# imuncle/TSCM_Calib

Measured on AMD Instinct MI355X. Metric: LM iterations/sec at 4 cams x 10k views (joint intrinsics+extrinsics, fp64), higher is better.
Workload: dtype f64

## Files before the change

### tscm_calib_amd/csrc/tscm_kernels.h

```cpp
#pragma once

#include "tscm_math.h"
#include "tscm_fastmath.h"
#include "tscm_nd_plan.h"
#include "tscm_layout.h"
#include "tscm_exec_plan.h"
#include "tscm_columns.h"
#include "tscm_ctrl.h"

namespace tscm {

static_assert(kColFree == kFA && kColGrad == kFR, "tscm_columns.h plans the columns of tscm_math.h's camera tile");
constexpr int kWcolTc = 3;
constexpr int kFac = 56;
constexpr int kFacM = 0;
constexpr int kFacC = 15;
constexpr int kFacL = 21;
constexpr int kFacI = 36;
constexpr int kFacZ = 42;
constexpr int kFacD = 48;
constexpr int kTcols = 15;
constexpr int kTcWb = 0, kTcWc = 4, kTcF = 8, kTcOne = 9, kTcXi = 10, kTcLam = 12, kTcAl = 13, kTcR = 14;
__host__ __device__ constexpr int tc_tc(int j) { return 3 + 4 * j; }
constexpr int kVConst = 27;
constexpr int kCConst = 48;
constexpr int kCStride = 72;
constexpr int kCst = 80;
constexpr int kScal = 8;
constexpr int kStStride = 16;

#if defined(TSCM_PHASE_PROFILE) || defined(TSCM_WAVE_TIMELINE)
#define PHASE_STAMP(var) const long long var = wall_clock64()
#else
#define PHASE_STAMP(var)
#endif

__device__ __forceinline__ void wave_lds_fence()
{
    __builtin_amdgcn_fence(__ATOMIC_RELEASE, "wavefront");
    __builtin_amdgcn_wave_barrier();
    __builtin_amdgcn_fence(__ATOMIC_ACQUIRE, "wavefront");
}

typedef int v2i __attribute__((ext_vector_type(2)));
__device__ __forceinline__ __amdgpu_buffer_rsrc_t make_rsrc(const void *p, size_t bytes)
{
    return __builtin_amdgcn_make_buffer_rsrc(const_cast<void *>(p), 0, (int)(bytes > 0xffffffffull ? 0xffffffffu : (unsigned)bytes), 0x00020000);
}
__device__ __forceinline__ double buf_load_f64(__amdgpu_buffer_rsrc_t r, unsigned voff, unsigned soff)
{
    return __builtin_bit_cast(double, __builtin_amdgcn_raw_buffer_load_b64(r, (int)voff, (int)soff, 0));
}
#ifndef TSCM_STORE_AUX
#define TSCM_STORE_AUX 0
#endif
__device__ __forceinline__ void buf_store_f64(__amdgpu_buffer_rsrc_t r, unsigned voff, unsigned soff, double v)
{
    __builtin_amdgcn_raw_buffer_store_b64(__builtin_bit_cast(v2i, v), r, (int)voff, (int)soff, TSCM_STORE_AUX);
}

typedef double d4 __attribute__((ext_vector_type(4)));
typedef double d2 __attribute__((ext_vector_type(2)));
typedef int v4i __attribute__((ext_vector_type(4)));
__device__ __forceinline__ d2 buf_load_2f64(__amdgpu_buffer_rsrc_t r, unsigned voff, unsigned soff)
{
    return __builtin_bit_cast(d2, __builtin_amdgcn_raw_buffer_load_b128(r, (int)voff, (int)soff, 0));
}
__device__ __forceinline__ void buf_store_2f64(__amdgpu_buffer_rsrc_t r, unsigned voff, double a, double b)
{
    const d2 v = { a, b };
    __builtin_amdgcn_raw_buffer_store_b128(__builtin_bit_cast(v4i, v), r, (int)voff, 0, TSCM_STORE_AUX);
}

#ifndef TSCM_PRIO
#define TSCM_PRIO 10
#endif
__device__ __forceinline__ void set_prio(int p)
{
    switch (p & 3) {
    case 0: __builtin_amdgcn_s_setprio(0); break;
    case 1: __builtin_amdgcn_s_setprio(1); break;
    case 2: __builtin_amdgcn_s_setprio(2); break;
    default: __builtin_amdgcn_s_setprio(3); break;
    }
}

__device__ __forceinline__ const double *rec_w(const double *rec, int slot) { return rec + (size_t)kRecW * slot; }
__device__ __forceinline__ const double *rec_e(const double *rec, int V, int slot) { return rec + (size_t)kRecW * V + (size_t)kRecE * slot; }
__device__ __forceinline__ const double *rec_g(const double *rec, int V, int slot) { return rec + (size_t)(kRecW + kRecE) * V + (size_t)kRecG * slot; }

struct Ctrl : CtrlHead {
    IterLog log[kMaxLog];
};

struct DevProblem {
    int C, B, n_points, V, N, n_pad;
    int n_chunks, n_pchunks, n_bids;
    int rp, half;
    int lds_wave;
    const double *board_xy;
    const int *view_cam, *view_board, *view_obs, *view_count;
    const double *obs_u, *obs_v;
    const int *chunk_vb, *chunk_ve, *chunk_cam, *cam_chunk_ptr;
    const int4 *chunk_desc;
    const int *bv_ptr;
    const int *view_slot, *slot_cam;
    const int *slot_view, *slot_board;
    const int *slow_boards;
    int n_slow;
    const int *pair_i, *pair_j;
    const int *pc_begin, *pc_end, *pc_tile;
    const int *bid_part_ptr;
    const int *pair_board;
    const int *bc_tile;
    const int4 *bc_desc;
    int n_bchunks, n_tiles;
    const unsigned char *col_ctl;
    const unsigned char *board_const;
    const unsigned char *col_active;
    const int *act_map;
    int n_act;
    int cam_pre[9];
    unsigned short cam_free[8];
    unsigned long long pair_mask;
    const int4 *solve_map;
    int cam_wg[9];
    int rank, world;
    const short *bid_lut;
    int bid_part_small[kSmallBids + 1];
    int g4_per;
};

struct DevState {
    double *cam_rt[2], *intr[2], *board_rt[2];
    double *board_pc, *cam_pc;
    double *vconst;
    double *cconst[2];
    double *rec[2];
    double *campart, *campart2;
    double *H[2], *H_stage;
    double *s_b, *s_c;
    double *fac;
    double *pairpart, *T;
    int *t_count;
    int *fac_fail;
    int *y_flag;
    double *yhat;
    double *Abig;
    double *bs_part, *st_part;
    int n_bs_blocks, n_st_blocks;
    Ctrl *ctrl;
    CtrlHead *ctrl_snap;
    int *stats_count, *stats_flag;
    struct CtlPub *ctl_pub;
};
struct CtlPub { int epoch, cur, done, pad; double radius; };

__global__ void k_pose_prep(DevProblem P, DevState S, int cand)
{
    if (S.ctrl->done) return;
    const int tgt = cand ? (S.ctrl->cur ^ 1) : S.ctrl->cur;
    const int i = blockIdx.x * blockDim.x + threadIdx.x;
    if (i < P.B) {
        double rt[6], out[kBoardConst];
        for (int k = 0; k < 6; ++k) rt[k] = S.board_rt[tgt][6 * i + k];
        board_constants(rt, out);
        for (int k = 0; k < kBoardConst; ++k) S.board_pc[(size_t)kBoardConst * i + k] = out[k];
    } else if (i < P.B + P.C) {
        const int m = i - P.B;
        double rt[6], out[kCamConst];
        for (int k = 0; k < 6; ++k) rt[k] = S.cam_rt[tgt][6 * m + k];
        camera_constants(rt, out);
        for (int k = 0; k < kCamConst; ++k) S.cam_pc[kCamConst * m + k] = out[k];
    }
}

__device__ __forceinline__ void load_view_const(const DevProblem &P, const DevState &S, int tgt, int cam, int board, ViewConst &vc)
{
    const double *bp = S.board_pc + (size_t)kBoardConst * board;
    for (int k = 0; k < 3; ++k) { vc.r1[k] = bp[k]; vc.r2[k] = bp[3 + k]; vc.tb[k] = S.board_rt[tgt][6 * board + 3 + k]; }
    for (int k = 0; k < 3; ++k) for (int q = 0; q < 6; ++q) vc.db[k][q] = bp[6 + 6 * k + q];
    const double *cp = S.cam_pc + kCamConst * cam;
    for (int k = 0; k < 9; ++k) vc.Rc[k] = cp[k];
    for (int k = 0; k < 27; ++k) vc.dRc[k] = cp[9 + k];
    for (int k = 0; k < 3; ++k) vc.tc[k] = S.cam_rt[tgt][6 * cam + 3 + k];
    const double *I = S.intr[tgt] + 9 * cam;
    vc.fx = I[0]; vc.fy = I[1]; vc.cx = I[2]; vc.cy = I[3]; vc.xi = I[4]; vc.lam = I[5]; vc.al = I[6];
}

__device__ __forceinline__ void view_point_constants(const double Rc[9], const double *tc, const double *bc , const double *tb, double *o)
{
    for (int r = 0; r < 3; ++r) {
        o[r] = Rc[3 * r] * bc[0] + Rc[3 * r + 1] * bc[1] + Rc[3 * r + 2] * bc[2];
        o[3 + r] = Rc[3 * r] * bc[3] + Rc[3 * r + 1] * bc[4] + Rc[3 * r + 2] * bc[5];
        o[6 + r] = (Rc[3 * r] * tb[0] + Rc[3 * r + 1] * tb[1] + Rc[3 * r + 2] * tb[2]) + tc[r];
    }
}

#if defined(__HIP_DEVICE_COMPILE__) && !defined(__gfx950__) && !defined(__gfx942__)
#error "the in-launch hand-offs (handoff_store / handoff_load) rely on gfx942 / gfx950 sc1 write-through semantics: re-derive them for this target"
#endif
constexpr long long kHandoffTimeoutTicks = 50 * 1000 * 1000;
__device__ __forceinline__ void handoff_store(double *p, double v) { __hip_atomic_store(p, v, __ATOMIC_RELAXED, __HIP_MEMORY_SCOPE_AGENT); }
__device__ __forceinline__ double handoff_load(const double *p) { return __hip_atomic_load(p, __ATOMIC_RELAXED, __HIP_MEMORY_SCOPE_AGENT); }

__device__ __forceinline__ void write_camera_record(const DevState &S, int tgt, int m, const double *cam_rt, const double *intr)
{
    double crt[3], Rc[9], a[9], wsm[3];
    for (int k = 0; k < 3; ++k) crt[k] = cam_rt[6 * m + k];
    const int small = camera_rotation_constants(crt, Rc, a, wsm);
    double *o = S.cconst[tgt] + kCStride * m;
    for (int k = 0; k < 9; ++k) o[k] = Rc[k];
    for (int k = 0; k < 3; ++k) o[9 + k] = cam_rt[6 * m + 3 + k];
    for (int k = 0; k < 9; ++k) o[12 + k] = a[k];
    for (int k = 0; k < 3; ++k) o[21 + k] = wsm[k];
    o[24] = small ? 1.0 : 0.0;
    for (int k = 25; k < 39; ++k) o[k] = 0.0;
    double I[7];
    for (int k = 0; k < 7; ++k) I[k] = intr[9 * m + k];
    for (int k = 0; k < 6; ++k) o[39 + k] = I[k];
    const double oma = 1.0 - I[6];
    o[45] = I[6] / oma;
    o[46] = 1.0 / (oma * oma);
    o[47] = 0.0;
    float *of = reinterpret_cast<float *>(o + kCConst);
    for (int k = 0; k < kCConst; ++k) of[k] = (float)o[k];
}
__device__ __forceinline__ void write_camera_record(const DevState &S, int tgt, int m) { write_camera_record(S, tgt, m, S.cam_rt[tgt], S.intr[tgt]); }

constexpr int kVStride = 48;
constexpr int kVFloatOff = 32;

__device__ __forceinline__ void view_prep_body(const DevProblem &P, const DevState &S, int tgt, int with_floats, const double *cam_rt, const double *intr, const double *board_rt)
{
    __shared__ double st[kVPrepThreads][kVFloatOff + 1];
    const int t = threadIdx.x;
    const int i = blockIdx.x * kVPrepThreads + t;
    if (i < P.V) {
        const int b = P.view_board[i], m = P.view_cam[i];
        double rt[6], bc[kBoardConst], Rc[9], dRc[27];
        for (int k = 0; k < 6; ++k) rt[k] = board_rt[6 * b + k];
        board_constants(rt, bc);
        double crt[3];
        for (int k = 0; k < 3; ++k) crt[k] = cam_rt[6 * m + k];
        rotation_and_derivatives(crt, Rc, dRc);
        double *o = st[t];
        view_point_constants(Rc, cam_rt + 6 * m + 3, bc, rt + 3, o);
        for (int k = 0; k < 6; ++k) {
            const double d0 = bc[6 + 3 * k], d1 = bc[6 + 3 * k + 1], d2 = bc[6 + 3 * k + 2];
            for (int r = 0; r < 3; ++r) o[9 + 3 * k + r] = Rc[3 * r] * d0 + Rc[3 * r + 1] * d1 + Rc[3 * r + 2] * d2;
        }
        for (int k = kVConst; k < kVFloatOff; ++k) o[k] = 0.0;
    } else if (i < P.V + P.C) {
        write_camera_record(S, tgt, i - P.V, cam_rt, intr);
    }
    __syncthreads();
    const int v0 = blockIdx.x * kVPrepThreads;
    const int nv = min(kVPrepThreads, P.V - v0);
    for (int e = t; e < nv * kVFloatOff; e += kVPrepThreads) {
        const int v = e / kVFloatOff, k = e % kVFloatOff;
        S.vconst[(size_t)kVStride * (v0 + v) + k] = st[v][k];
    }
    if (with_floats) {
        constexpr int kF = kVStride - kVFloatOff;
        for (int e = t; e < nv * kF; e += kVPrepThreads) {
            const int v = e / kF, k = e % kF, j = 2 * k;
            const float f0 = j < kVConst ? (float)st[v][j] : 0.f, f1 = j + 1 < kVConst ? (float)st[v][j + 1] : 0.f;
            S.vconst[(size_t)kVStride * (v0 + v) + kVFloatOff + k] = __hiloint2double(__float_as_int(f1), __float_as_int(f0));
        }
    }
}

__global__ __launch_bounds__(kVPrepThreads) void k_view_prep(DevProblem P, DevState S, int cand, int with_floats)
{
    if (S.ctrl->done) return;
    const int tgt = cand ? (S.ctrl->cur ^ 1) : S.ctrl->cur;
    view_prep_body(P, S, tgt, with_floats, S.cam_rt[tgt], S.intr[tgt], S.board_rt[tgt]);
}

__host__ __device__ __forceinline__ constexpr int f_tile(int f)
{
    return f < 3 ? kTcWc + f : f < 6 ? tc_tc(f - 3) : f < 8 ? kTcF : f < 10 ? kTcOne : f == 10 ? kTcXi : f == 11 ? kTcLam : f == 12 ? kTcAl : kTcR;
}
__device__ __forceinline__ int f_mask(int f) { return (f >= 6 && f < 10) ? (1 << ((f - 6) & 1)) : 3; }

typedef const double __attribute__((address_space(4))) *cptr4;

struct RecLane { unsigned off, stride, goff, gstride; };
__device__ __forceinline__ RecLane rec_lane(int lane, unsigned V)
{
    const int col = lane & 15, kq = lane >> 4;
    RecLane r;
    r.goff = col == kTcR ? 8u * ((unsigned)(kRecW + kRecE) * V + (unsigned)kq) : 0xffffe000u; r.gstride = col == kTcR ? 8u * kRecG : 0u;
    if (col < 3) { r.off = 8u * ((unsigned)kRecW * V + 6u * (unsigned)col + (unsigned)kq); r.stride = 8u * kRecE; }
    else if (col == 15) { r.off = 0xffffe000u; r.stride = 0u; }
    else {
        const int f = (col & 3) == 3 ? kWcolTc + (col >> 2) : col < 8 ? col - kTcWc : col == kTcF ? 6 : col == kTcOne ? 8 : col == kTcXi ? 10 : col - 1;
        r.off = 8u * (6u * (unsigned)f + (unsigned)kq); r.stride = 8u * kRecW;
    }
    return r;
}

template <typename PW, typename PR>
__host__ __device__ __forceinline__ double tb_tb(PW W, PR Rc, int l, int lp)
// ... 1285 lines not shown
#pragma unroll
            for (int b = 0; b < kFA; ++b) o.hrow[b] = H[256 * m + ai * 16 + b];
            o.hg = H[256 * m + ai * 16 + kFR];
        }
    }
}
__device__ __forceinline__ void reduced_solution_tail(const DevProblem &P, const DevState &S, int cur, int fail, const TailOperands &o,
                                                      const double *yv, const double *s_sc, double *s_yh, const unsigned char *s_act, double *sred,
                                                      int publish_epoch = 0)
{
    const int n = P.n_pad, i = threadIdx.x;
    const int m = i >> 4, ai = i & 15;
    double model = 0.0, stepsq = 0.0, yh = 0.0;
    if (i < n) {
        const bool act = s_act[i] && !fail;
        yh = act ? s_sc[i] * yv[i] : 0.0;
        handoff_store(&S.yhat[i], yh);
        s_yh[i] = yh;
        if (ai < kFA) {
            const double x = o.x;
            const double xn = x + (-yh);
            if (ai < 6) handoff_store(&S.cam_rt[cur ^ 1][6 * m + ai], xn); else handoff_store(&S.intr[cur ^ 1][9 * m + (ai - 6)], xn);
            const double d = x - xn; stepsq = d * d;
        } else if (ai < 15) {
            handoff_store(&S.intr[cur ^ 1][9 * m + (ai - 6)], o.x);
        }
    }
    if (publish_epoch > 0) asm volatile("s_waitcnt vmcnt(0)" ::: "memory");
    __syncthreads();
    if (publish_epoch > 0 && i == 0) __hip_atomic_store(S.y_flag, 2 * publish_epoch + (fail ? 1 : 0), __ATOMIC_RELAXED, __HIP_MEMORY_SCOPE_AGENT);
    if (publish_epoch > 0 && i >= 64 && i < 64 + P.C) write_camera_record(S, cur ^ 1, i - 64);
    if (i < n && ai < kFA && yh != 0.0) {
        double hy = 0.0;
#pragma unroll
        for (int b = 0; b < kFA; ++b) hy += o.hrow[b] * s_yh[m * 16 + b];
        model = yh * (o.hg - 0.5 * hy);
    }
    { double red[2] = { model, stepsq }, mdummy = 0.0; block_reduce256<2>(red, mdummy, sred); model = red[0]; stepsq = red[1]; }
    if (i == 0) { S.ctrl->model_cam = model; S.ctrl->stepsq_cam = stepsq; S.ctrl->lin_fail = fail; *S.fac_fail = 0; }
}

template <int NTH, bool WAIT>
__device__ __forceinline__ void backsub_body(const DevProblem &P, const DevState &S, int with_floats, const int blk, const int nblk, const int epoch, const int t_need);

#include "tscm_solve_nd.h"
#include "tscm_solve_dense4.h"

constexpr int kBigNT = 1024;
constexpr int kBigBatch = 4;
__host__ __device__ inline size_t solve_big_lds_bytes(int N, int n_pad)
{
    return sizeof(double) * ((size_t)2 * 16 * (N + 16) + 16 * 17 + 2 * (size_t)N + 16 + 3 * (size_t)n_pad) + sizeof(int) * (size_t)N + (size_t)n_pad;
}
__device__ __forceinline__ size_t big_block(int I, int J) { return ((size_t)(I * (I + 1) / 2 + J)) << 8; }
__device__ __forceinline__ size_t big_idx(int r, int c)
{
    return big_block(r >> 4, c >> 4) + (size_t)((((c & 15) + 16 * (r & 3)) << 2) + ((r & 15) >> 2));
}
__device__ __forceinline__ double readlane_f64(double v, int lane)
{
    return __hiloint2double(__builtin_amdgcn_readlane(__double2hiint(v), lane), __builtin_amdgcn_readlane(__double2loint(v), lane));
}
__device__ __forceinline__ void lds_barrier() { asm volatile("s_waitcnt lgkmcnt(0)\n\ts_barrier" ::: "memory"); }

__global__ __launch_bounds__(kBigNT) void k_solve_reduced_big(DevProblem P, DevState S)
{
    extern __shared__ __attribute__((aligned(32))) double lds[];
    const int n = P.n_pad, na = P.n_act;
    const int N = (na + 15) & ~15, NP = N >> 4;
    const int XP = N + 16;
    double *pbuf = lds;
    double *Ld = pbuf + 2 * 16 * XP;
    double *wv = Ld + 16 * 17;
    double *idg = wv + N;
    double *yk = idg + N;
    double *yv = yk + 16;
    double *s_sc = yv + n;
    double *s_yh = s_sc + n;
    int *s_map = reinterpret_cast<int *>(s_yh + n);
    unsigned char *s_act = reinterpret_cast<unsigned char *>(s_map + N);
    __shared__ int s_fail;
    __shared__ double sred[256];
    const int tid = threadIdx.x, wave = tid >> 6, lane = tid & 63;
    if (S.ctrl->done) return;
    const int cur = S.ctrl->cur;
    const double radius = S.ctrl->radius;
    const double dmin = S.ctrl->opt.min_lm_diagonal, dmax = S.ctrl->opt.max_lm_diagonal;
    const double *H = S.H[cur];
    double *A = S.Abig;
    for (int i = tid; i < n; i += kBigNT) { s_sc[i] = S.s_c[i]; s_act[i] = P.col_active[i]; yv[i] = 0.0; }
    for (int i = tid; i < N; i += kBigNT) s_map[i] = i < na ? P.act_map[i] : -1;
    if (tid == 0) s_fail = S.ctrl->lin_fail | *S.fac_fail;
    __syncthreads();
#ifdef TSCM_BIG_PROFILE
    long long tp0 = wall_clock64(), tp_diag = 0, tp_solve = 0, tp_upd = 0;
#endif
    for (int kb = 0; wave + 16 * kb <= N; kb += 16) {
        const int rmax = min(N, wave + 16 * (kb + 15));
        for (int c = lane; c <= rmax && c < N; c += 64) {
            const int j = s_map[c];
            const int mj = j >> 4, bj = j & 15;
            const double scj = j >= 0 ? s_sc[j] : 0.0;
            double v[16];
#pragma unroll
            for (int u = 0; u < 16; ++u) {
                const int r = wave + 16 * (kb + u);
                v[u] = (r == c) ? 1.0 : 0.0;
                if (r > N || c > r) continue;
                if (r == N) {
                    v[u] = j >= 0 ? scj * (H[256 * mj + bj * 16 + kFR] - load_T_lut(P, S.T, j, mj * 16 + kFR)) : 0.0;
                } else {
                    const int i = s_map[r];
                    if (i >= 0 && j >= 0) {
                        const int mi = i >> 4, ai = i & 15;
                        const double h = (mi == mj) ? H[256 * mi + ai * 16 + bj] : 0.0;
                        double t = s_sc[i] * scj * (h - load_T_lut(P, S.T, i, j));
                        if (i == j) t += fmin(fmax(scj * scj * h, dmin), dmax) / radius;
                        v[u] = t;
                    }
                }
            }
#pragma unroll
            for (int u = 0; u < 16; ++u) {
                const int r = wave + 16 * (kb + u);
                if (r > N || c > r) continue;
                if (c < 16) pbuf[c * XP + r] = v[u];
                else A[big_idx(r, c)] = v[u];
            }
        }
    }
    __syncthreads();
#ifdef TSCM_BIG_PROFILE
    long long tp1 = wall_clock64();
#endif
    for (int tk = 0; tk < NP; ++tk) {
        const int k0 = tk * 16, m0 = k0 + 16;
        double *pc = pbuf + (tk & 1) * (16 * XP);
        double *pn = pbuf + ((tk & 1) ^ 1) * (16 * XP);
#ifdef TSCM_BIG_PROFILE
        const long long q0 = wall_clock64();
#endif
        if (wave == 0) {
            const int r = lane & 15;
            double a[16];
#pragma unroll
            for (int c = 0; c < 16; ++c) a[c] = pc[c * XP + r];
#pragma unroll
            for (int c = 0; c < 16; ++c) {
                double d = readlane_f64(a[c], c);
                if (!(d > 0.0)) { d = 1.0; if (lane == 0) s_fail = 1; }
                const double isd = fast_rsqrt(d);
                const double l = a[c] * isd;
                a[c] = l;
                if (lane == c) idg[k0 + c] = isd;
#pragma unroll
                for (int q = c + 1; q < 16; ++q) a[q] -= l * readlane_f64(l, q);
            }
            if (lane < 16) {
#pragma unroll
                for (int c = 0; c < 16; ++c) if (c <= r) { Ld[r * 17 + c] = a[c]; A[big_idx(k0 + r, k0 + c)] = a[c]; }
            }
        }
        lds_barrier();
#ifdef TSCM_BIG_PROFILE
        const long long q1 = wall_clock64();
#endif
        for (int r = m0 + tid; r <= N; r += kBigNT) {
            double x[16];
#pragma unroll
            for (int c = 0; c < 16; ++c) x[c] = pc[c * XP + (r - k0)];
#pragma unroll
            for (int c = 0; c < 16; ++c) {
                double v = x[c];
#pragma unroll
                for (int q = 0; q < c; ++q) v -= x[q] * Ld[c * 17 + q];
                x[c] = v * idg[k0 + c];
            }
#pragma unroll
            for (int c = 0; c < 16; ++c) { A[big_idx(r, k0 + c)] = x[c]; pc[c * XP + (r - k0)] = x[c]; }
        }
        lds_barrier();
#ifdef TSCM_BIG_PROFILE
        const long long q2 = wall_clock64();
#endif
        {
            const int col = lane & 15, kq = lane >> 4;
            const int Tb = tk + 1;
            for (int I = Tb + (((wave >> 2) - Tb) & 3); I <= NP; I += 4) {
                double xa[4];
#pragma unroll
                for (int t = 0; t < 4; ++t) xa[t] = -pc[(4 * t + kq) * XP + (16 * I - k0) + col];
                for (int J0 = Tb + (((wave & 3) - Tb) & 3); J0 <= I && J0 < NP; J0 += 4 * kBigBatch) {
                    d4 acc[kBigBatch];
#pragma unroll
                    for (int u = 0; u < kBigBatch; ++u) {
                        const int J = J0 + 4 * u;
                        const int Jc = (J <= I && J < NP) ? J : J0;
                        acc[u] = *reinterpret_cast<const d4 *>(A + big_block(I, Jc) + 4 * lane);
                    }
#pragma unroll
                    for (int u = 0; u < kBigBatch; ++u) {
                        const int J = J0 + 4 * u;
                        if (!(J <= I && J < NP)) continue;
                        double xb[4];
#pragma unroll
                        for (int t = 0; t < 4; ++t) xb[t] = pc[(4 * t + kq) * XP + (16 * J - k0) + col];
#pragma unroll
                        for (int t = 0; t < 4; ++t) acc[u] = __builtin_amdgcn_mfma_f64_16x16x4f64(xa[t], xb[t], acc[u], 0, 0, 0);
                    }
#pragma unroll
                    for (int u = 0; u < kBigBatch; ++u) {
                        const int J = J0 + 4 * u;
                        if (!(J <= I && J < NP)) continue;
                        if (J == Tb) {
#pragma unroll
                            for (int g = 0; g < 4; ++g) pn[col * XP + 16 * (I - Tb) + kq + 4 * g] = acc[u][g];
                        } else {
                            *reinterpret_cast<d4 *>(A + big_block(I, J) + 4 * lane) = acc[u];
                        }
                    }
                }
            }
        }
        lds_barrier();
#ifdef TSCM_BIG_PROFILE
        { const long long q3 = wall_clock64(); tp_diag += q1 - q0; tp_solve += q2 - q1; tp_upd += q3 - q2; }
#endif
    }
    __syncthreads();
#ifdef TSCM_BIG_PROFILE
    long long tp2 = wall_clock64();
#endif
    for (int i = tid; i < N; i += kBigNT) wv[i] = A[big_idx(N, i)];
    double lrow[16], ldg[4];
    {
        const int k0 = (NP - 1) * 16;
#pragma unroll
        for (int c = 0; c < 16; ++c) lrow[c] = (NP > 0 && tid < k0) ? A[big_idx(k0 + c, tid)] : 0.0;
#pragma unroll
        for (int u = 0; u < 4; ++u) { const int e = lane + 64 * u, r = e >> 4, c = e & 15; ldg[u] = (NP > 0 && wave == 0 && c <= r) ? A[big_idx(k0 + r, k0 + c)] : 0.0; }
    }
    __syncthreads();
    for (int tk = NP - 1; tk >= 0; --tk) {
        const int k0 = tk * 16;
        double lnext[16], dnext[4];
        {
            const int kn = k0 - 16;
#pragma unroll
            for (int c = 0; c < 16; ++c) lnext[c] = (tk > 0 && tid < kn) ? A[big_idx(kn + c, tid)] : 0.0;
#pragma unroll
            for (int u = 0; u < 4; ++u) { const int e = lane + 64 * u, r = e >> 4, c = e & 15; dnext[u] = (tk > 0 && wave == 0 && c <= r) ? A[big_idx(kn + r, kn + c)] : 0.0; }
        }
        if (wave == 0) {
#pragma unroll
            for (int u = 0; u < 4; ++u) { const int e = lane + 64 * u; Ld[(e >> 4) * 17 + (e & 15)] = ldg[u]; }
            wave_lds_fence();
            if (lane == 0) {
                double y[16];
#pragma unroll
                for (int c = 15; c >= 0; --c) {
                    double v = wv[k0 + c];
#pragma unroll
                    for (int q = c + 1; q < 16; ++q) v -= Ld[q * 17 + c] * y[q];
                    y[c] = v * idg[k0 + c];
                }
#pragma unroll
                for (int c = 0; c < 16; ++c) { yk[c] = y[c]; wv[k0 + c] = y[c]; }
            }
        }
        lds_barrier();
        if (tid < k0) {
            double v = wv[tid];
#pragma unroll
            for (int c = 0; c < 16; ++c) v -= lrow[c] * yk[c];
            wv[tid] = v;
        }
        lds_barrier();
#pragma unroll
        for (int c = 0; c < 16; ++c) lrow[c] = lnext[c];
#pragma unroll
        for (int u = 0; u < 4; ++u) ldg[u] = dnext[u];
    }
    TailOperands tail_ops;
    tail_prefetch(P, S, cur, H, tail_ops);
    for (int i = tid; i < na; i += kBigNT) yv[s_map[i]] = wv[i];
    __syncthreads();
#ifdef TSCM_BIG_PROFILE
    long long tp3 = wall_clock64();
#endif
    reduced_solution_tail(P, S, cur, s_fail, tail_ops, yv, s_sc, s_yh, s_act, sred);
#ifdef TSCM_BIG_PROFILE
    if (tid == 0) printf("big solve N=%d  build %lld  factor %lld (diag %lld solve %lld update %lld)  backsub %lld  tail %lld  [10 ns ticks]\n", N,
                         tp1 - tp0, tp2 - tp1, tp_diag, tp_solve, tp_upd, tp3 - tp2, wall_clock64() - tp3);
#endif
}

constexpr int kBsTile = 64;
template <int NTH> struct BsGeom {
    static constexpr int kBoards = NTH / 8;
    static constexpr int kPassSlots = NTH / 16;
    static constexpr int kPasses = 4;
    static constexpr int kRoundSlots = kPasses * kPassSlots;
    static constexpr int kLdsA = kRoundSlots * 6, kLdsB = kBoards * kFac, kLdsC = kBsTile * (kVFloatOff + 1);
    static constexpr int kLds = kLdsC > kLdsB ? (kLdsC > kLdsA ? kLdsC : kLdsA) : (kLdsB > kLdsA ? kLdsB : kLdsA);
    static_assert(kBoards * kFac == 7 * NTH, "the factor records are 7 doubles per thread");
    static_assert(kBoards <= 64 && 64 + kMaxCam <= NTH, "lane roles of phase B: the boards in wave 0, the cameras from wave 1 on");
};

template <int NTH, bool WAIT>
__device__ __forceinline__ void backsub_body(const DevProblem &P, const DevState &S, int with_floats, const int blk, const int nblk, const int epoch, const int t_need)
{
    constexpr int kBsBoards = BsGeom<NTH>::kBoards, kBsThreads = NTH, kPassSlots = BsGeom<NTH>::kPassSlots, kPasses = BsGeom<NTH>::kPasses, kRoundSlots = BsGeom<NTH>::kRoundSlots;
#ifndef TSCM_BS_CAM_LANE0
#define TSCM_BS_CAM_LANE0 64
#endif
    constexpr int kBsCamLane0 = TSCM_BS_CAM_LANE0;
    const int b0 = blk * kBsBoards;
    const int nbl = min(kBsBoards, P.B - b0);
    const int s0 = P.bv_ptr[b0], s1 = P.bv_ptr[b0 + nbl];
    const int ctrl_done = S.ctrl->done, cur = S.ctrl->cur;
    int fail = WAIT ? 0 : S.ctrl->lin_fail;
    if (ctrl_done) return;
    extern __shared__ __attribute__((aligned(16))) double dyn[];
    double (*s_qv)[6] = reinterpret_cast<double (*)[6]>(dyn);
    double *s_fac = dyn;
    double *st_all = dyn;
    __shared__ double s_q[kBsBoards][6], s_new[kBsBoards][6];
    __shared__ double s_yh[16 * kMaxCam];
    double (*s_rc)[12] = reinterpret_cast<double (*)[12]>(s_yh);
    static_assert(12 * kMaxCam <= 16 * kMaxCam, "s_rc aliases s_yh");
    __shared__ double sm[16];
    __shared__ int s_view[kBsTile];
    const int t = threadIdx.x;
    PHASE_STAMP(ts0);
    const int my_q0 = t < nbl ? P.bv_ptr[b0 + t] : 0, my_q1 = t < nbl ? P.bv_ptr[b0 + t + 1] : 0;
    const int c_slot = min(s0 + t, max(s1 - 1, 0));
    const int c_view = s1 > s0 ? P.slot_view[c_slot] : 0, c_board = s1 > s0 ? P.slot_board[c_slot] : 0, c_cam = s1 > s0 ? P.slot_cam[c_slot] : 0;
    double xb[6], sbv[6];
#pragma unroll
    for (int k = 0; k < 6; ++k) { xb[k] = t < nbl ? S.board_rt[cur][6 * (b0 + t) + k] : 0.0; sbv[k] = t < nbl ? S.s_b[6 * (b0 + t) + k] : 1.0; }
    double facv[7];
#pragma unroll
    for (int j = 0; j < 7; ++j) facv[j] = S.fac[(size_t)kFac * b0 + min(t + kBsThreads * j, nbl * kFac - 1)];
    if constexpr (!WAIT) { for (int i = t; i < P.n_pad; i += kBsThreads) s_yh[i] = S.yhat[i]; }
    if (t < kBsBoards * 6) (&s_q[0][0])[t] = 0.0;
    if constexpr (!WAIT) { if (t == 64) for (int m = blk; m < P.C; m += nblk) write_camera_record(S, cur ^ 1, m); }
    {
        const int grp = t >> 4, a = t & 15;
        const __amdgpu_buffer_rsrc_t r_w = make_rsrc(S.rec[cur], sizeof(double) * (size_t)kRecW * P.V);
        constexpr unsigned BAD = 0xffffe000u;
        double w[kPasses][6];
        int camv[kPasses];
        auto request = [&](int rbase) {
#pragma unroll
            for (int j = 0; j < kPasses; ++j) {
                const int slot = rbase + kPassSlots * j + grp;
                const unsigned off = (a < kFA && slot < s1) ? 8u * ((unsigned)kRecW * (unsigned)slot + 6u * (unsigned)a) : BAD;
#pragma unroll
                for (int k = 0; k < 3; ++k) { const d2 v = buf_load_2f64(r_w, off, 16u * (unsigned)k); w[j][2 * k] = v[0]; w[j][2 * k + 1] = v[1]; }
                camv[j] = P.slot_cam[min(slot, max(s1 - 1, 0))];
            }
        };
        request(s0);
        if constexpr (WAIT) {
            __shared__ int s_flag;
            if (t == 0) {
                const long long t_start = wall_clock64();
                int f;
                while (((f = __hip_atomic_load(S.y_flag, __ATOMIC_RELAXED, __HIP_MEMORY_SCOPE_AGENT)) >> 1) < epoch) {
                    __builtin_amdgcn_s_sleep(8);
                    if (wall_clock64() - t_start > kHandoffTimeoutTicks) { f = -1; break; }
                }
                if (f < 0) {
                    __hip_atomic_store(&S.ctrl->fault, 1, __ATOMIC_RELAXED, __HIP_MEMORY_SCOPE_AGENT);
                    __hip_atomic_store(&S.ctrl->term_type, 2, __ATOMIC_RELAXED, __HIP_MEMORY_SCOPE_AGENT);
                    __hip_atomic_store(&S.ctrl->done, 1, __ATOMIC_RELAXED, __HIP_MEMORY_SCOPE_AGENT);
                }
                s_flag = f;
            }
            __syncthreads();
            if (s_flag < 0 || __hip_atomic_load(&S.ctrl->done, __ATOMIC_RELAXED, __HIP_MEMORY_SCOPE_AGENT)) return;
            fail = s_flag & 1;
            for (int i = t; i < P.n_pad; i += kBsThreads) s_yh[i] = handoff_load(&S.yhat[i]);
        }
        for (int rbase = s0; rbase < s1; rbase += kRoundSlots) {
            const int rend = min(s1, rbase + kRoundSlots);
            __syncthreads();
#pragma unroll
            for (int j = 0; j < kPasses; ++j) {
                const int sl = kPassSlots * j + grp;
                const double yh = a < kFA ? s_yh[16 * camv[j] + a] : 0.0;
                double p[6];
#pragma unroll
                for (int k = 0; k < 6; ++k) {
                    p[k] = (a < kFA ? w[j][k] : 0.0) * yh;
                    p[k] = row16_allsum(p[k]);
                }
                if (a == 0) {
#pragma unroll
                    for (int k = 0; k < 6; ++k) s_qv[sl][k] = p[k];
                }
            }
            if (rbase + kRoundSlots < s1) request(rbase + kRoundSlots);
            __syncthreads();
            if (t < nbl) {
                for (int q = max(my_q0, rbase); q < min(my_q1, rend); ++q)
#pragma unroll
                    for (int k = 0; k < 6; ++k) s_q[t][k] += s_qv[q - rbase][k];
            }
        }
        __syncthreads();
#pragma unroll
        for (int j = 0; j < 7; ++j) s_fac[t + kBsThreads * j] = facv[j];
        __syncthreads();
    }
    PHASE_STAMP(ts1);
    double mb = 0.0, ss = 0.0;
    if (t < nbl) {
        const int b = b0 + t;
        if (my_q1 == my_q0 || fail) {
#pragma unroll
            for (int k = 0; k < 6; ++k) { S.board_rt[cur ^ 1][6 * b + k] = xb[k]; s_new[t][k] = xb[k]; }
        } else {
            const double *f = s_fac + kFac * t;
            double tt[6], y[6], pz[6];
#pragma unroll
            for (int i = 0; i < 6; ++i) {
                double v = f[kFacC + i] * s_q[t][i];
#pragma unroll
                for (int k = 0; k < i; ++k) v -= f[kFacM + i * (i - 1) / 2 + k] * pz[k];
                pz[i] = v;
                tt[i] = f[kFacZ + i] - v;
            }
#pragma unroll
            for (int i = 5; i >= 0; --i) {
                double w = tt[i];
#pragma unroll
                for (int k = i + 1; k < 6; ++k) w -= f[kFacL + k * (k - 1) / 2 + i] * y[k];
                y[i] = w * f[kFacI + i];
            }
#pragma unroll
            for (int k = 0; k < 6; ++k) {
                mb += 0.5 * tt[k] * tt[k] + 0.5 * f[kFacD + k] * y[k] * y[k];
                const double x = xb[k];
                const double xn = x + (-(sbv[k] * y[k]));
                const double d = x - xn;
                ss += d * d;
                S.board_rt[cur ^ 1][6 * b + k] = xn;
                s_new[t][k] = xn;
            }
        }
    } else if (t >= kBsCamLane0 && t < kBsCamLane0 + P.C) {
        const int m = t - kBsCamLane0;
        double crt[3], Rc[9], dRc[27];
        double crt6[6];
#pragma unroll
        for (int k = 0; k < 6; ++k) crt6[k] = WAIT ? handoff_load(&S.cam_rt[cur ^ 1][6 * m + k]) : S.cam_rt[cur ^ 1][6 * m + k];
        for (int k = 0; k < 3; ++k) crt[k] = crt6[k];
        rotation_and_derivatives(crt, Rc, dRc);
        for (int k = 0; k < 9; ++k) s_rc[m][k] = Rc[k];
        for (int k = 0; k < 3; ++k) s_rc[m][9 + k] = crt6[3 + k];

    }
    {
        double red[2] = { mb, ss }, mdummy = 0.0;
        block_reduce256<2>(red, mdummy, sm);
        if (t == 0) { S.bs_part[2 * blk] = red[0]; S.bs_part[2 * blk + 1] = red[1]; }
    }
    PHASE_STAMP(ts2);
    for (int base = s0; base < s1; base += kBsTile) {
        const int slot = base + t;
        int view = -1;
        if (t < kBsTile && slot < s1) {
            const bool first = base == s0;
            view = first ? c_view : P.slot_view[slot];
            const int bl = (first ? c_board : P.slot_board[slot]) - b0, m = first ? c_cam : P.slot_cam[slot];
            double rt[6], bc[kBoardConst];
#pragma unroll
            for (int k = 0; k < 6; ++k) rt[k] = s_new[bl][k];
            board_constants(rt, bc);
            double *o = st_all + (size_t)t * (kVFloatOff + 1);
            view_point_constants(s_rc[m], s_rc[m] + 9, bc, rt + 3, o);
            for (int k = 0; k < 6; ++k) {
                const double d0 = bc[6 + 3 * k], d1 = bc[6 + 3 * k + 1], d2 = bc[6 + 3 * k + 2];
                for (int r = 0; r < 3; ++r) o[9 + 3 * k + r] = s_rc[m][3 * r] * d0 + s_rc[m][3 * r + 1] * d1 + s_rc[m][3 * r + 2] * d2;
            }
            for (int k = kVConst; k < kVFloatOff; ++k) o[k] = 0.0;
        }
        if (t < kBsTile) s_view[t] = view;
        __syncthreads();
        const int nrec = min(kBsTile, s1 - base);
        for (int e = t; e < nrec * kVFloatOff; e += kBsThreads) {
            const int v = e / kVFloatOff, k = e % kVFloatOff;
            S.vconst[(size_t)kVStride * s_view[v] + k] = st_all[(size_t)v * (kVFloatOff + 1) + k];
        }
        if (with_floats) {
            constexpr int kF = kVStride - kVFloatOff;
            for (int e = t; e < nrec * kF; e += kBsThreads) {
                const int v = e / kF, k = e % kF, j = 2 * k;
                const double *sv = st_all + (size_t)v * (kVFloatOff + 1);
                const float f0 = j < kVConst ? (float)sv[j] : 0.f, f1 = j + 1 < kVConst ? (float)sv[j + 1] : 0.f;
                S.vconst[(size_t)kVStride * s_view[v] + kVFloatOff + k] = __hiloint2double(__float_as_int(f1), __float_as_int(f0));
            }
        }
        __syncthreads();
    }
#ifdef TSCM_WAVE_TIMELINE
    if (threadIdx.x == 0 && S.ctrl->iteration == 5 && blk < kKtlGroups) {
        long long *o = g_phs + (size_t)kPhStamps * (kKtlGroups + blk);
        o[0] = ts0; o[1] = ts0; o[2] = ts1; o[3] = ts2; o[4] = wall_clock64(); o[5] = o[4]; o[6] = nbl; o[7] = 0;
    }
#endif
#ifdef TSCM_PHASE_PROFILE
    if (threadIdx.x == 0 && (blk == 0 || blk == 200))
        printf("backsub_prep wg %d: W.yhat %lld  board solve %lld  view constants %lld [10 ns]\n", blk, ts1 - ts0, ts2 - ts1, wall_clock64() - ts2);
#endif
}

template <int NTH>
__global__ __launch_bounds__(NTH) void k_backsub_prep(DevProblem P, DevState S, int with_floats)
{
    KTL(5);
    backsub_body<NTH, false>(P, S, with_floats, (int)blockIdx.x, (int)gridDim.x, 0, 0);
}

__device__ void control_step(const DevProblem &P, const DevState &S, int init, const ControlPre &pre, double *sm, const double *H, const double *sc, double *stage_copy,
                             bool writer, CtlOut *out)
{
    Ctrl &g = *S.ctrl;
    CtrlHead c = pre.c;
    const int t = threadIdx.x;
    if (out && t == 0) { out->cur = c.cur; out->done = c.done; out->radius = c.radius; out->dmin = c.opt.min_lm_diagonal; out->dmax = c.opt.max_lm_diagonal; }
    if (c.done) return;
    const Options &o = c.opt;
    const int tgt = init ? c.cur : (c.cur ^ 1);
    double gmax_c = 0.0, gsq_c = 0.0, xsq_c = 0.0, cost = 0.0;
#pragma unroll
    for (int j = 0; j < 2; ++j) {
        const int p = t + 256 * j;
        if (p >= 16 * P.C) break;
        const int m = p >> 4, a = p & 15;
        if (pre.free_param[j]) {
            const double x = pre.x[j];
            const double g = pre.grad_param[j] ? H[256 * m + a * 16 + kFR] : 0.0;
            const double d = x - (x + (-g));
            gmax_c = fmax(gmax_c, fabs(d)); gsq_c += d * d; xsq_c += x * x;
        }
        if (a == 15) cost += 0.5 * H[256 * m + kFR * 16 + kFR];
        if (init && writer && a < 15) {
            const double hii = (a < kFA) ? H[256 * m + a * 16 + a] : 0.0;
            S.s_c[p] = o.jacobi_scaling ? 1.0 / (1.0 + sqrt(hii)) : 1.0;
        }
        if (init && writer && a == 15) S.s_c[p] = 1.0;
    }
    KTLX(4, true);
    { double red[3] = { gsq_c, xsq_c, cost }; block_reduce256<3>(red, gmax_c, sm); gsq_c = red[0]; xsq_c = red[1]; cost = red[2]; }
    KTLX(5, true);
    if (writer) {
#pragma unroll 8
        for (int i = t; i < 256 * P.C; i += 256) { const double h = H[i]; S.H[tgt][i] = h; if (stage_copy) stage_copy[i] = h; }
        if (stage_copy && t < kScal + P.world) stage_copy[256 * P.C + t] = sc[t];
    }
    if (t != 0) return;
    auto commit = [&]() {
        c.fin_count = 0;
        if (writer) static_cast<CtrlHead &>(g) = c;
        if (out) { out->cur = c.cur; out->done = c.done; out->radius = c.radius; }
    };
    double gmax_b = 0.0;
    for (int r = 0; r < P.world; ++r) gmax_b = fmax(gmax_b, sc[kScal + r]);
    const double gmax_t = fmax(gmax_c, gmax_b);
    if (sc[4] > 0.0) c.lin_fail = 1;
    const double gnorm_t = sqrt(gsq_c + sc[3]);
    const double xnorm_t = sqrt(xsq_c + sc[2]);
    KTLX(6, true);

    IterLog it;
    const StepInput in = { cost, gmax_t, gnorm_t, xnorm_t, sc[0] + c.model_cam, sqrt(sc[1] + c.stepsq_cam) };
    if (lm_step(c, init, tgt, in, it) && writer && c.n_log <= kMaxLog) g.log[c.n_log - 1] = it;
    commit();
}

__global__ __launch_bounds__(256) void k_control(DevProblem P, DevState S, int init)
{
    __shared__ double sm[256];
    ControlPre pre;
    control_prefetch(P, S, init, pre, S.ctrl);
    control_step(P, S, init, pre, sm, S.H_stage, S.H_stage + 256 * P.C, nullptr);
}

__global__ __launch_bounds__(kVPrepThreads) void k_begin_view_prep(DevProblem P, DevState S, CtrlHead head, const double *src_cam, const double *src_intr,
                                                                   const double *src_board, double *bak_cam, double *bak_intr, double *bak_board, int with_floats)
{
    const int i0 = blockIdx.x * kVPrepThreads + threadIdx.x, n = gridDim.x * kVPrepThreads;
    if (i0 == 0) { head.t_begin = wall_clock64(); static_cast<CtrlHead &>(*S.ctrl) = head; }
    if (i0 == 0) { *S.t_count = 0; *S.y_flag = 0; *S.fac_fail = 0; S.ctl_pub->epoch = 0; *S.stats_count = 0; *S.stats_flag = 0; }
    const double *cam = src_cam ? src_cam : S.cam_rt[0], *intr = src_intr ? src_intr : S.intr[0], *board = src_board ? src_board : S.board_rt[0];
    for (int i = i0; i < 6 * P.C; i += n) { const double v = cam[i]; if (src_cam) S.cam_rt[0][i] = v; if (bak_cam) bak_cam[i] = v; }
    for (int i = i0; i < 9 * P.C; i += n) { const double v = intr[i]; if (src_intr) S.intr[0][i] = v; if (bak_intr) bak_intr[i] = v; }
    for (int i = i0; i < 6 * P.B; i += n) { const double v = board[i]; if (src_board) S.board_rt[0][i] = v; if (bak_board) bak_board[i] = v; }
    view_prep_body(P, S, 0, with_floats, cam, intr, board);
}

__global__ __launch_bounds__(256) void k_end_solve(DevState S, int C, int B)
{
    const int i0 = blockIdx.x * 256 + threadIdx.x, n = gridDim.x * 256;
    if (i0 == 0) S.ctrl->t_end = wall_clock64();
    if (S.ctrl->cur == 0) return;
    for (int i = i0; i < 6 * C; i += n) S.cam_rt[0][i] = S.cam_rt[1][i];
    for (int i = i0; i < 9 * C; i += n) S.intr[0][i] = S.intr[1][i];
    for (int i = i0; i < 6 * B; i += n) S.board_rt[0][i] = S.board_rt[1][i];
}

__global__ __launch_bounds__(256) void k_finish_solve(DevProblem P, DevState S, int init, int have_backsub, int C, int B, Ctrl *host_ctrl)
{
    constexpr int kHl = 256 * kMaxCamLds + kScal + 8, kGall = 512 * kMaxCamLds;
    __shared__ double sm[256];
    __shared__ double Hl[kHl];
    __shared__ CtlOut s_ctl;
    const CtrlHead *head = S.ctrl_snap;
    if (blockIdx.x == 0) {
        __shared__ double Gall[kGall];
        finish_evaluation<false>(P, S, init, have_backsub, true, Hl, Gall, sm, &s_ctl, head);
        __syncthreads();
        if (threadIdx.x == 0) S.ctrl->t_end = wall_clock64();
        __threadfence();
        __syncthreads();
        const int n_log = min(max(__hip_atomic_load(&S.ctrl->n_log, __ATOMIC_RELAXED, __HIP_MEMORY_SCOPE_AGENT), 0), kMaxLog);
        const int words = (int)((sizeof(CtrlHead) + sizeof(IterLog) * (size_t)n_log) / 8);
        const unsigned long long *src = reinterpret_cast<const unsigned long long *>(S.ctrl);
        unsigned long long *dst = reinterpret_cast<unsigned long long *>(host_ctrl);
        for (int i = threadIdx.x; i < words; i += 256) dst[i] = __hip_atomic_load(&src[i], __ATOMIC_RELAXED, __HIP_MEMORY_SCOPE_AGENT);
        return;
    }
    control_outcome(P, S, init, have_backsub, Hl, sm, &s_ctl, head);
    __syncthreads();
    if (__builtin_amdgcn_readfirstlane(s_ctl.cur) == 0) return;
    const int i0 = (blockIdx.x - 1) * 256 + threadIdx.x, n = (gridDim.x - 1) * 256;
    for (int i = i0; i < 6 * C; i += n) S.cam_rt[0][i] = S.cam_rt[1][i];
    for (int i = i0; i < 9 * C; i += n) S.intr[0][i] = S.intr[1][i];
    for (int i = i0; i < 6 * B; i += n) S.board_rt[0][i] = S.board_rt[1][i];
}

__global__ void k_eval_functor(DevProblem P, DevState S, const int *corner_view, double *res,
                               double *Jc, double *Jb, double *Ji)
{
    const int k = blockIdx.x * blockDim.x + threadIdx.x;
    if (k >= P.N) return;
    const int view = corner_view[k];
    const int j = k - P.view_obs[view];
    ViewConst vc;
    load_view_const(P, S, 0, P.view_cam[view], P.view_board[view], vc);
    double r[2], JE[2][kE], JF[2][kFA];
    corner_residual_jacobian(vc, P.board_xy[2 * j], P.board_xy[2 * j + 1], P.obs_u[k], P.obs_v[k], r, JE, JF);
    res[2 * k] = r[0]; res[2 * k + 1] = r[1];
    for (int row = 0; row < 2; ++row) {
        if (Jc) for (int i = 0; i < 6; ++i) Jc[12 * (size_t)k + 6 * row + i] = JF[row][i];
        if (Jb) for (int i = 0; i < 6; ++i) Jb[12 * (size_t)k + 6 * row + i] = JE[row][i];
        if (Ji) { for (int i = 0; i < 7; ++i) Ji[18 * (size_t)k + 9 * row + i] = JF[row][6 + i]; Ji[18 * (size_t)k + 9 * row + 7] = 0.0; Ji[18 * (size_t)k + 9 * row + 8] = 0.0; }
    }
}

__global__ __launch_bounds__(64) void k_reproj_error(DevProblem P, const double *cam_rt, const double *intr,
                                                    const double *board_rt, double *view_err, double *view_sq)
{
    const int view = blockIdx.x, lane = threadIdx.x;
    const int cam = P.view_cam[view], board = P.view_board[view];
    double Rb[9], Rc[9], dummy[27], I[9];
    rotation_and_derivatives(board_rt + 6 * board, Rb, dummy);
    rotation_and_derivatives(cam_rt + 6 * cam, Rc, dummy);
    for (int i = 0; i < 9; ++i) I[i] = intr[9 * cam + i];
    const double *tb = board_rt + 6 * board + 3, *tc = cam_rt + 6 * cam + 3;
    double e = 0.0, sq = 0.0;
    for (int j = lane; j < P.view_count[view]; j += 64) {
        const double x = P.board_xy[2 * j], y = P.board_xy[2 * j + 1];
        double q[3], Pc[3];
        for (int i = 0; i < 3; ++i) q[i] = Rb[3 * i] * x + Rb[3 * i + 1] * y + tb[i];
        for (int i = 0; i < 3; ++i) Pc[i] = Rc[3 * i] * q[0] + Rc[3 * i + 1] * q[1] + Rc[3 * i + 2] * q[2] + tc[i];
        double u, v;
        project_point(I, Pc[0], Pc[1], Pc[2], u, v);
        const double du = P.obs_u[P.view_obs[view] + j] - u, dv = P.obs_v[P.view_obs[view] + j] - v;
        e += sqrt(du * du + dv * dv); sq += du * du + dv * dv;
    }
    for (int s = 32; s > 0; s >>= 1) { e += __shfl_xor(e, s); sq += __shfl_xor(sq, s); }
    if (lane == 0) { view_err[view] = e; view_sq[view] = sq; }
}

__global__ void k_project(const double *intr, const double *pts, int n, double *uv)
{
    const int i = blockIdx.x * blockDim.x + threadIdx.x;
    if (i >= n) return;
    double I[9];
    for (int k = 0; k < 9; ++k) I[k] = intr[k];
    project_point(I, pts[3 * i], pts[3 * i + 1], pts[3 * i + 2], uv[2 * i], uv[2 * i + 1]);
}

__global__ void k_unproject(const double *intr, const double *uv, int n, double *rays)
{
    const int i = blockIdx.x * blockDim.x + threadIdx.x;
    if (i >= n) return;
    double I[9], r[3];
    for (int k = 0; k < 9; ++k) I[k] = intr[k];
    unproject_pixel(I, uv[2 * i], uv[2 * i + 1], r);
    rays[3 * i] = r[0]; rays[3 * i + 1] = r[1]; rays[3 * i + 2] = r[2];
}

}
```

Baseline: 8718.

## Split view-record construction across waves and precompute board constants once per board

```diff
diff --git a/tscm_calib_amd/csrc/tscm_kernels.h b/tscm_calib_amd/csrc/tscm_kernels.h
--- a/tscm_calib_amd/csrc/tscm_kernels.h
+++ b/tscm_calib_amd/csrc/tscm_kernels.h
@@ -1,5 +1,6 @@
 #pragma once
 
+#include <type_traits>
 #include "tscm_math.h"
 #include "tscm_fastmath.h"
 #include "tscm_nd_plan.h"
@@ -1891,10 +1892,30 @@
     static constexpr int kPasses = 4;
     static constexpr int kRoundSlots = kPasses * kPassSlots;
     static constexpr int kLdsA = kRoundSlots * 6, kLdsB = kBoards * kFac, kLdsC = kBsTile * (kVFloatOff + 1);
-    static constexpr int kLds = kLdsC > kLdsB ? (kLdsC > kLdsA ? kLdsC : kLdsA) : (kLdsB > kLdsA ? kLdsB : kLdsA);
+    static constexpr int kLdsABC = kLdsC > kLdsB ? (kLdsC > kLdsA ? kLdsC : kLdsA) : (kLdsB > kLdsA ? kLdsB : kLdsA);
+    static constexpr int kBcPitch = kBoardConst + 1, kLdsBc = kBoards * kBcPitch;
+    static constexpr int kLds = kLdsABC + kLdsBc;
+    static constexpr int kWaves = NTH / 64;
+    static constexpr int kBcWave = kWaves >= 3 ? 2 : 0, kPoseWave = kWaves - 1;
     static_assert(kBoards * kFac == 7 * NTH, "the factor records are 7 doubles per thread");
     static_assert(kBoards <= 64 && 64 + kMaxCam <= NTH, "lane roles of phase B: the boards in wave 0, the cameras from wave 1 on");
+    static_assert(kBcWave != 1 && kPoseWave != kBcWave, "the board constants are formed next to the camera rotations (wave 1) and the pose stores");
 };
+template <int NW> struct BsRoles;
+template <> struct BsRoles<4> { static constexpr int kLo[5] = { 0, 9, 15, 21, kVConst }; };
+template <> struct BsRoles<2> { static constexpr int kLo[3] = { 0, 15, kVConst }; };
+template <int NW> constexpr bool bs_roles_cover()
+{
+    int seen[kVConst] = {};
+    for (int w = 0; w < NW; ++w) {
+        const int lo = BsRoles<NW>::kLo[w], hi = BsRoles<NW>::kLo[w + 1];
+        if (lo % 3 || hi % 3 || (lo > 0 && lo < 9)) return false;
+        for (int k = lo; k < hi; ++k) { if (k < 0 || k >= kVConst) return false; ++seen[k]; }
+    }
+    for (int k = 0; k < kVConst; ++k) if (seen[k] != 1) return false;
+    return true;
+}
+static_assert(bs_roles_cover<4>() && bs_roles_cover<2>(), "every output 0 .. 26 of a view record belongs to exactly one wave");
 
 template <int NTH, bool WAIT>
 __device__ __forceinline__ void backsub_body(const DevProblem &P, const DevState &S, int with_floats, const int blk, const int nblk, const int epoch, const int t_need)
@@ -1914,6 +1935,8 @@
     double (*s_qv)[6] = reinterpret_cast<double (*)[6]>(dyn);
     double *s_fac = dyn;
     double *st_all = dyn;
+    double *s_bc = dyn + BsGeom<NTH>::kLdsABC;
+    constexpr int kBcPitch = BsGeom<NTH>::kBcPitch, kWaves = BsGeom<NTH>::kWaves;
     __shared__ double s_q[kBsBoards][6], s_new[kBsBoards][6];
     __shared__ double s_yh[16 * kMaxCam];
     double (*s_rc)[12] = reinterpret_cast<double (*)[12]>(s_yh);
@@ -1921,10 +1944,15 @@
     __shared__ double sm[16];
     __shared__ int s_view[kBsTile];
     const int t = threadIdx.x;
+    const int wv = __builtin_amdgcn_readfirstlane(t >> 6), ln = t & 63;
     PHASE_STAMP(ts0);
     const int my_q0 = t < nbl ? P.bv_ptr[b0 + t] : 0, my_q1 = t < nbl ? P.bv_ptr[b0 + t + 1] : 0;
-    const int c_slot = min(s0 + t, max(s1 - 1, 0));
-    const int c_view = s1 > s0 ? P.slot_view[c_slot] : 0, c_board = s1 > s0 ? P.slot_board[c_slot] : 0, c_cam = s1 > s0 ? P.slot_cam[c_slot] : 0;
+    int c_view = 0, c_board = 0, c_cam = 0, n_view = 0, n_board = 0, n_cam = 0;
+    auto request_tile = [&](int base, int &view, int &board, int &cam) {
+        const int slot = min(base + ln, s1 - 1);
+        view = P.slot_view[slot]; board = P.slot_board[slot]; cam = P.slot_cam[slot];
+    };
+    if (s1 > s0) { request_tile(s0, c_view, c_board, c_cam); request_tile(s0 + kBsTile, n_view, n_board, n_cam); }
     double xb[6], sbv[6];
 #pragma unroll
     for (int k = 0; k < 6; ++k) { xb[k] = t < nbl ? S.board_rt[cur][6 * (b0 + t) + k] : 0.0; sbv[k] = t < nbl ? S.s_b[6 * (b0 + t) + k] : 1.0; }
@@ -2006,10 +2034,9 @@
     PHASE_STAMP(ts1);
     double mb = 0.0, ss = 0.0;
     if (t < nbl) {
-        const int b = b0 + t;
         if (my_q1 == my_q0 || fail) {
 #pragma unroll
-            for (int k = 0; k < 6; ++k) { S.board_rt[cur ^ 1][6 * b + k] = xb[k]; s_new[t][k] = xb[k]; }
+            for (int k = 0; k < 6; ++k) s_new[t][k] = xb[k];
         } else {
             const double *f = s_fac + kFac * t;
             double tt[6], y[6], pz[6];
@@ -2035,7 +2062,6 @@
                 const double xn = x + (-(sbv[k] * y[k]));
                 const double d = x - xn;
                 ss += d * d;
-                S.board_rt[cur ^ 1][6 * b + k] = xn;
                 s_new[t][k] = xn;
             }
         }
@@ -2051,31 +2077,55 @@
         for (int k = 0; k < 3; ++k) s_rc[m][9 + k] = crt6[3 + k];
 
     }
+    __syncthreads();
+    if (wv == BsGeom<NTH>::kBcWave && ln < nbl) {
+        double rt[6], bc[kBoardConst];
+#pragma unroll
+        for (int k = 0; k < 6; ++k) rt[k] = s_new[ln][k];
+        board_constants(rt, bc);
+#pragma unroll
+        for (int k = 0; k < kBoardConst; ++k) s_bc[kBcPitch * ln + k] = bc[k];
+    }
+    if (wv == BsGeom<NTH>::kPoseWave) {
+        for (int i = ln; i < 6 * nbl; i += 64) S.board_rt[cur ^ 1][6 * b0 + i] = (&s_new[0][0])[i];
+    }
     {
         double red[2] = { mb, ss }, mdummy = 0.0;
         block_reduce256<2>(red, mdummy, sm);
         if (t == 0) { S.bs_part[2 * blk] = red[0]; S.bs_part[2 * blk + 1] = red[1]; }
     }
     PHASE_STAMP(ts2);
+    auto view_outputs = [&](auto role, int bl, int m) {
+        constexpr int lo = BsRoles<kWaves>::kLo[decltype(role)::value], hi = BsRoles<kWaves>::kLo[decltype(role)::value + 1];
+        const double *bc = s_bc + kBcPitch * bl;
+        double *o = st_all + (size_t)ln * (kVFloatOff + 1);
+        if constexpr (lo == 0) {
+            double tb[3];
+#pragma unroll
+            for (int k = 0; k < 3; ++k) tb[k] = s_new[bl][3 + k];
+            view_point_constants(s_rc[m], s_rc[m] + 9, bc, tb, o);
+        }
+        for (int k = (lo > 9 ? lo - 9 : 0) / 3; k < (hi - 9) / 3; ++k) {
+            const double d0 = bc[6 + 3 * k], d1 = bc[6 + 3 * k + 1], d2 = bc[6 + 3 * k + 2];
+            for (int r = 0; r < 3; ++r) o[9 + 3 * k + r] = s_rc[m][3 * r] * d0 + s_rc[m][3 * r + 1] * d1 + s_rc[m][3 * r + 2] * d2;
+        }
+        if constexpr (hi == kVConst) { for (int k = kVConst; k < kVFloatOff; ++k) o[k] = 0.0; }
+    };
     for (int base = s0; base < s1; base += kBsTile) {
-        const int slot = base + t;
+        const int slot = base + ln;
         int view = -1;
-        if (t < kBsTile && slot < s1) {
-            const bool first = base == s0;
-            view = first ? c_view : P.slot_view[slot];
-            const int bl = (first ? c_board : P.slot_board[slot]) - b0, m = first ? c_cam : P.slot_cam[slot];
-            double rt[6], bc[kBoardConst];
-#pragma unroll
-            for (int k = 0; k < 6; ++k) rt[k] = s_new[bl][k];
-            board_constants(rt, bc);
-            double *o = st_all + (size_t)t * (kVFloatOff + 1);
-            view_point_constants(s_rc[m], s_rc[m] + 9, bc, rt + 3, o);
-            for (int k = 0; k < 6; ++k) {
-                const double d0 = bc[6 + 3 * k], d1 = bc[6 + 3 * k + 1], d2 = bc[6 + 3 * k + 2];
-                for (int r = 0; r < 3; ++r) o[9 + 3 * k + r] = s_rc[m][3 * r] * d0 + s_rc[m][3 * r + 1] * d1 + s_rc[m][3 * r + 2] * d2;
-            }
-            for (int k = kVConst; k < kVFloatOff; ++k) o[k] = 0.0;
-        }
+        if (slot < s1) {
+            view = c_view;
+            const int bl = c_board - b0, m = c_cam;
+            if (wv == 0) view_outputs(std::integral_constant<int, 0>{}, bl, m);
+            else if (wv == 1) view_outputs(std::integral_constant<int, 1>{}, bl, m);
+            if constexpr (kWaves == 4) {
+                if (wv == 2) view_outputs(std::integral_constant<int, 2>{}, bl, m);
+                else if (wv == 3) view_outputs(std::integral_constant<int, 3>{}, bl, m);
+            }
+        }
+        c_view = n_view; c_board = n_board; c_cam = n_cam;
+        if (base + 2 * kBsTile < s1) request_tile(base + 2 * kBsTile, n_view, n_board, n_cam);
         if (t < kBsTile) s_view[t] = view;
         __syncthreads();
         const int nrec = min(kBsTile, s1 - base);
```

Result: no change. 8696, median of 2 (-0.3%).
